# mjlaine/mcmcf90

Measured on AMD Instinct MI355X. Metric: MH proposals/sec (whole node), d=50 Gaussian target, higher is better.
Workload: dtype f64

## Files before the change

### mcmcf90_amd/csrc/mcx_api.hip

```cpp
#include <hip/hip_runtime.h>
#include <csignal>
#include <cmath>
#include <cstdio>
#include <cstdlib>
#include <cstring>
#include <string>
#include <vector>
#include <algorithm>
#include "../../include/mcmcx.h"
#include "../../include/mcmcx_target.h"
#include "mcx_kernels.hpp"
#include "mcx_group.hpp"
#include "mcx_group_ram.hpp"

#include "mcx_host_engine.hpp"
#include "mcx_host_linalg.hpp"
#include "mcx_host_launch.hpp"
#include "mcx_host_adapt.hpp"
#include "mcx_host_pooled.hpp"
#include "mcx_host_callbacks.hpp"

extern "C" {

const char *mcmcx_last_error(void) { return g_err.c_str(); }
// ... 316 lines not shown
    E.ny = h->ny; E.hs = h->d + h->ny;
    E.alphatarget = c.alphatarget; E.drscale = c.drscale; E.scalelimit = c.scalelimit; E.scalefactor = c.scalefactor;
    E.k0 = c.seed; E.chain_id0 = c.chain_id0;
    E.dr_lds = h->plan.dr_lds ? 1 : 0;
    E.lds_scratch = h->plan.lds_form;
    E.tgt.kind = phased(h) ? (int)TGT_HOST : h->tkind;
    E.tgt.b = h->tb; E.tgt.ndata = (int)h->tx.size(); E.tgt.ncols = h->tncols;
    const int d = h->d;
    int rc;
    if (h->tkind == TGT_GAUSS) {
        if ((rc = dev_upload(h, &E.tgt.mu, h->tmu))) return rc;
        std::vector<double> lt((size_t)(d + 4) * d + 64, 0.0);
        for (int i = 0; i < d; ++i) for (int j = 0; j < d; ++j) lt[(size_t)j * d + i] = h->tlam[(size_t)i * d + j];
        if ((rc = dev_upload(h, &E.tgt.lamT, lt))) return rc;
    }
    if (h->tkind == TGT_EXPDATA || h->tkind == TGT_EXPCOLS) { if ((rc = dev_upload(h, &E.tgt.x, h->tx))) return rc; if ((rc = dev_upload(h,
        &E.tgt.y, h->ty))) return rc; }
    if (h->has_lo && (rc = dev_upload(h, &E.tgt.lo, h->tlo))) return rc;
    if (h->has_hi && (rc = dev_upload(h, &E.tgt.hi, h->thi))) return rc;
    if (h->has_pri) { if ((rc = dev_upload(h, &E.tgt.pmu, h->tpmu))) return rc; if ((rc = dev_upload(h, &E.tgt.psig, h->tpsig))) return rc;
        }
    if ((rc = dev_upload(h, &E.par0, h->par0))) return rc;
    return dev_upload(h, &E.cmat0p, f.Cp);
}
static int init_chains(mcmcx_engine *h, const InitialFactor &f)
{
    const mcmcx_config &c = h->cfg;
    EngineDev &E = h->E;
    const int d = h->d, P = h->P, T = h->ntiles, ny = h->ny;
    const size_t L = (size_t)T * 64, DD = (size_t)d * d;
    int rc;
    if ((rc = dev_alloc(h, &E.theta, L * d))) return rc;
    if ((rc = h->plan.host_mapped ? host_alloc(h, &E.cand, L * d) : dev_alloc(h, &E.cand, L * d))) return rc;
    if ((rc = dev_alloc(h, &E.zs, L * 2 * d))) return rc;
    if ((rc = h->plan.cs_mapped ? host_alloc(h, &E.cs, L * 2 * d) : dev_alloc(h, &E.cs, L * 2 * d))) return rc;
    if (h->plan.xscr && (rc = dev_alloc(h, &E.xscr, L * 2 * d))) return rc;
    if ((rc = dev_alloc(h, &E.scal, L * NSCAL))) return rc;
    if ((rc = dev_alloc(h, &E.ictr, L * NICTR))) return rc;
    if ((rc = dev_alloc(h, &E.rngn, L))) return rc;
    if (!h->pooled && (rc = dev_alloc(h, &E.R, L * P, false))) return rc;
    if ((rc = dev_alloc(h, &E.basetheta, L * d))) return rc;
    if (h->usesvd && !h->pooled) {
        if ((rc = dev_alloc(h, &E.Rf, L * DD, false))) return rc;
        if (c.method != MCMCX_METHOD_RAM) {
            if ((rc = dev_alloc(h, &E.Gw, L * DD)) || (rc = dev_alloc(h, &E.Vw, L * DD))) return rc;
            if (h->plan.svd_blocked && ((rc = dev_alloc(h, &h->d_Gc, L * DD, false)) || (rc = dev_alloc(h, &h->d_Vc, L * DD, false))
                || (rc = dev_alloc(h, &h->d_svc, L * d, false)) || (rc = dev_alloc(h, &h->d_need, L)) || (rc = dev_alloc(h, &h->d_state, L))
                || (rc = dev_alloc(h, &h->d_anyrot, 1)))) return rc;
        }
        if ((rc = dev_alloc(h, &E.qstd, L * d))) return rc;
        if (h->dodr && (rc = dev_alloc(h, &E.R2f, L * DD, false))) return rc;
        if ((rc = dev_bcast(h, E.Rf, f.Rfull)) || (rc = dev_bcast(h, E.qstd, f.qstd))) return rc;
        if (h->dodr) {
            std::vector<double> r2 = f.Rfull;
            for (auto &v : r2) v = v / c.drscale;
            if ((rc = dev_bcast(h, E.R2f, r2))) return rc;
        }
    }
    if (h->dodr && !h->pooled && ((rc = dev_alloc(h, &E.R2, L * P, false)) || (rc = dev_alloc(h, &E.iC, L * P, false)))) return rc;
    const bool am = h->plan.am;
    h->wcap = 0;
    if (am || c.record_chain) {
        long long wc = (c.record_chain || (am && c.adapthist > 1)) ? (long long)c.nsimu + 1
                                      : (long long)c.burnintime + 2LL * c.adaptint + c.adapthist + 2;
        if (wc > (long long)c.nsimu + 1) wc = (long long)c.nsimu + 1;
        h->wcap = (int)wc;
        if ((rc = dev_alloc(h, &E.hist, L * (size_t)h->wcap * (d + ny), false))) return rc;
        if ((rc = dev_alloc(h, &E.wacc, (size_t)T * h->wcap))) return rc;
        if (c.record_chain && c.updatesigma) { E.record_s2 = 1; if ((rc = dev_alloc(h, &E.s2hist, L * (size_t)h->wcap * ny))) return rc; }
// ... 675 lines not shown
```

### mcmcf90_amd/csrc/mcx_common.hpp

```cpp
#pragma once
#include "mcx_device.hpp"
#include <type_traits>

namespace mcx {


enum { TGT_GAUSS = 0, TGT_BANANA = 1, TGT_EXPDATA = 2, TGT_HOST = 3, TGT_EXPCOLS = 4, TGT_MODULE = 5 };
enum { M_DRAM = 0, M_RAM = 1, M_ER = 3 };

enum { S_SS1 = 0, S_PRI1, S_SIGMA2, S_ALPHA12, S_SAVEDY, S_WSUM, S_WNEW, NSCAL };
enum { I_SAVED = 0, I_STAYED, I_BNDSTAYED, I_DRACC, I_DRTRIES, I_CHAININD, I_CURCOUNT, I_STATUS,
       I_LASTFREQ, I_BASECNT, I_WINSTART, I_INFO, I_ERSTAYED, I_PDESC, I_DOWNS, I_ADFLAGS, I_NR, I_BSTART, NICTR };

enum { ST_RAM_DOWNDATE_FAIL = 1, ST_CHOL_FAIL = 2, ST_POTRI_FAIL = 4 };

struct DevTarget {
    int kind;
    const double *mu, *lamT;
    double b;
    int ndata;
    const double *x, *y;
    int ncols;
    const double *lo, *hi;
    const double *pmu, *psig;
};

struct EngineDev {
    int d, P, ntiles;
    int method, dodr, updatesigma, doadapt, doburnin, burnintime, greedy, adapthist;
    double initcmatn;
    double gam_shape;
    double N0S02;
    double alphatarget, drscale, scalelimit, scalefactor;
    DevTarget tgt;
    double *theta, *cand, *zs, *cs, *scal, *R, *R2, *iC, *Rtmp;
    double *xscr;
    double *cmat, *mean, *basetheta;
    const double *cmat0p, *par0;
    uint32_t *ictr;
    uint64_t *rngn;
    uint32_t k0, chain_id0;
    int wcap, record_s2;
    double *hist, *s2hist;
    uint64_t *wacc;
    uint64_t *accmask;
    uint64_t *rowlist;
    const double *sharedR;
    int usesvd, doscam; double condmax;
    int scam_fast;
    double *Rf, *R2f, *qstd, *Gw, *Vw;
    double *hev, *hx;
    int ny, hs;
    double *ssv, *s2v, *ss2v;
    const double *gshapev;
    int lds_scratch;
    int dr_lds;
};

#define TIDX(base, tile, K, k, lane) ((base)[((size_t)(tile) * (size_t)(K) + (size_t)(k)) * 64 + (lane)])

MCX_DEV int rowstart(int i, int d) { return i * d - (i * (i - 1)) / 2; }
MCX_DEV int pidx(int i, int j, int d) { return rowstart(i, d) + (j - i); }

constexpr int CH = 8;

#define XL(j) X[(j) * 64 + lane]
#define GV(p, k) (p)[(size_t)(k) * 64 + lane]
#define GV2(p, k, c) (p)[(size_t)(k) * 64 + (c)]
#define LDNT(p, k) __builtin_nontemporal_load(&(p)[(size_t)(k) * 64 + lane])
// ... 423 lines not shown
```

### mcmcf90_amd/csrc/mcx_host_engine.hpp

```cpp

using namespace mcx;
static_assert(MCMCX_HE_INB == HE_INB && MCMCX_HE_PRI == HE_PRI && MCMCX_HE_SS == HE_SS && MCMCX_HX_STAGE2 == HX_STAGE2
    && MCMCX_HX_CRIT == HX_CRIT,
              "include/mcmcx_target.h and mcx_kernels.hpp disagree about the phase-state slots");

static thread_local std::string g_err;
static int fail(int code, const std::string &msg) { g_err = msg; return code; }

#define HIPCHK(call)                                                                              \
    do {                                                                                          \
        hipError_t e_ = (call);                                                                   \
        if (e_ != hipSuccess)                                                                     \
            return fail(-100, std::string(#call) + ": " + hipGetErrorString(e_));                 \
    } while (0)

struct mcx_switches {
    int pooled_mfma_dr_min = -1, pooled_scalar = -1, dr_big = -1, scam_pooled_16 = -1, scam_fast_lanes = -1, scam_waves = -1,
        svd_lane = -1, cov_batch_rows = -1, ram_wide = -1, pooled_waves = -1, pooled_ks = -1, cols_phased = -1, host_mapped = -1,
            host_fuse = -1, lds_scratch = -1, group = -1, group_dr2 = -1, group_gw = -1, ram_group = -1, tile_factor = -1,
            pooled_phase_mfma = -1;
    static int get(const char *name) { const char *e = getenv(name); return e ? atoi(e) : -1; }
    void read()
    {
        pooled_mfma_dr_min = get("MCMCX_POOLED_MFMA_DR_MIN"); pooled_scalar = get("MCMCX_POOLED_SCALAR"); dr_big = get("MCMCX_DR_BIG");
        scam_pooled_16 = get("MCMCX_SCAM_POOLED_16"); scam_fast_lanes = get("MCMCX_SCAM_FAST_LANES");
        scam_waves = get("MCMCX_SCAM_WAVES"); svd_lane = get("MCMCX_SVD_LANE"); cov_batch_rows = get("MCMCX_COV_BATCH_ROWS");
        ram_wide = get("MCMCX_RAM_WIDE"); pooled_waves = get("MCMCX_POOLED_WAVES"); pooled_ks = get("MCMCX_POOLED_KS");
        cols_phased = get("MCMCX_COLS_PHASED"); host_mapped = get("MCMCX_HOST_MAPPED"); host_fuse = get("MCMCX_HOST_FUSE");
        lds_scratch = get("MCMCX_LDS_SCRATCH"); group = get("MCMCX_GROUP"); group_dr2 = get("MCMCX_GROUP_DR2");
        group_gw = get("MCMCX_GROUP_GW"); ram_group = get("MCMCX_RAM_GROUP"); tile_factor = get("MCMCX_TILE_FACTOR");
        pooled_phase_mfma = get("MCMCX_POOLED_PHASE_MFMA");
    }
};
enum LdsForm { LDS_NONE = 0, LDS_STATE = 1, LDS_STATE_R = 2, LDS_RAM_R = 3 };
enum SharedLayout { SH_R = 1, SH_RT = 2, SH_DR = 4, SH_DRT = 8, SH_U = 16, SH_UREP = 32 };
struct KernelEntry;
struct KernelPlan {
    int lds_form = LDS_NONE;
    bool dr_lds = false;
    bool dr_vectors_in_lds = false;
    int group_d4 = 0, group_drm = 0, group_gw = 16;
    int ram_group_d4 = 0;
    bool tile_factor = false;
    bool svd_blocked = false;
    bool cov_batch = true;
    bool scam_replicated = false;
    bool host_mapped = false, cs_mapped = false;
    bool host_fuse = true;
    bool fused_cols = false;
    bool pooled_mfma = false;
    bool pooled_dr_mfma = false;
    bool pooled_two_waves = false, pooled_forty_rows = false;
    int pooled_phase = 0;
    bool ram_wide = false;
    bool scam_pooled12 = false, scam_fast_tile = false; int scam_waves = 1;
    bool am = false;
    bool xscr = false;
    unsigned shared = 0;
    const KernelEntry *step = nullptr;
    const KernelEntry *scam = nullptr;
};
struct PooledState {
    int status = 0; double alpha = 0.0;
    double W = 0.0; std::vector<double> mean, C, R;
    std::vector<double> Rf;
    std::vector<double> U, std;
    std::vector<double> R2, iC;
    double *d_R = nullptr;
    double *d_RT = nullptr;
    double *d_R2 = nullptr, *d_iC = nullptr;
    double *d_R2T = nullptr, *d_iCd = nullptr;
    double *d_U = nullptr;
};
struct mcmcx_engine {
    mcmcx_config cfg;
    KernelPlan plan;
    int d = 0, P = 0, ntiles = 0, nlanes = 0;
    int dodr = 0, usesvd = 0;
    bool inited = false;
    int simuind = 0;
    const char *last_kernel = "";
    std::string launch_err;
    std::vector<double> par0, cmat0;
    double sigma2 = 1.0; int nobs = 1; bool sigma2ok = false;
    int ny = 1; std::vector<double> sigma2v; std::vector<int> nobsv;
    int tkind = -1, tncols = 1; std::vector<double> tmu, tlam, tx, ty, tlo, thi, tpmu, tpsig; double tb = 0.1;
    bool has_lo = false, has_hi = false, has_pri = false;
// ... 94 lines not shown
```

### mcmcf90_amd/csrc/mcx_host_launch.hpp

```cpp

static size_t pooled_mfma_lds(int d)
{
    const size_t d4 = (size_t)((d + 3) & ~3), nt = (size_t)((d + 15) / 16);
    const size_t rows = (nt <= 4) ? std::max(d4, 4 * nt) : d4 + 16 * nt + 4 * nt;
    return rows * 64 * sizeof(double);
}
static bool pooled_use_mfma(const mcmcx_engine *h, const mcx_switches &sw)
{
    if (!h->pooled || (h->cfg.method != MCMCX_METHOD_DRAM && h->cfg.method != MCMCX_METHOD_RAM
        && h->cfg.method != MCMCX_METHOD_ER)) return false;
    if (h->dodr) {
        int dmin = 21;
        if (sw.pooled_mfma_dr_min >= 0) dmin = sw.pooled_mfma_dr_min;
        if (h->d < dmin) return false;
    }
    if (sw.pooled_scalar > 0) return false;
    return pooled_mfma_lds(h->d) <= 160 * 1024;
}
static bool phased(const mcmcx_engine *h) { return h->tkind == TGT_HOST || h->tkind == TGT_EXPCOLS || h->tkind == TGT_MODULE; }
static bool phase_cut(const mcmcx_engine *h) { return phased(h) && !h->plan.fused_cols; }
static int kernel_method(const mcmcx_engine *h)
{
    const int m = h->cfg.method;
    return (m == MCMCX_METHOD_RAM && !h->pooled) ? M_RAM : (m == MCMCX_METHOD_ER ? M_ER : M_DRAM);
}
static size_t lds_bytes(const mcmcx_engine *h) { return (size_t)h->d * 64 * sizeof(double) * 2; }
static bool dr_fits_lds(const mcmcx_engine *h) { return lds_bytes(h) <= 160 * 1024; }
static size_t lds_step(const mcmcx_engine *h) { return h->plan.dr_lds ? lds_bytes(h) : 0; }
static bool dr_vectors_in_lds(const mcmcx_engine *h, const mcx_switches &sw, int min_waves)
{
    if (!dr_fits_lds(h)) return false;
    if (sw.dr_big >= 0) return sw.dr_big == 0;
    return lds_bytes(h) * (size_t)min_waves <= 160 * 1024;
}
static void launch_init(mcmcx_engine *h)
{ hipLaunchKernelGGL(init_kernel, dim3(h->ntiles), dim3(64), 0, h->stream, h->E); }
struct KernelEntry {
    const char *family;
    const char *name;
    bool (*when)(const mcmcx_engine *);
    void (*launch)(mcmcx_engine *, int it0, int it1);
    unsigned shared = 0;
};
static const KernelEntry *pick_entry(const mcmcx_engine *h, const KernelEntry *tab, size_t n)
{
    for (size_t i = 0; i < n; ++i)
        if (tab[i].when(h)) return &tab[i];
    return nullptr;
}
static void launch_entry(mcmcx_engine *h, const KernelEntry *e, const char *family, int it0, int it1)
{
    if (!e) { h->launch_err = std::string("no ") + family + " kernel covers this configuration"; return; }
    h->last_kernel = e->name;
    e->launch(h, it0, it1);
}
static const int GROUP_MAXSEG = 256;
static const int GROUP_MAX_NPAR = 64, GROUP_MAX_NPAR_DR = 32;
static bool group_covers(const mcmcx_engine *h)
{
    const mcmcx_config &c = h->cfg;
    return !h->pooled && (c.method == MCMCX_METHOD_DRAM || (c.method == MCMCX_METHOD_ER && !h->dodr)) && !h->usesvd && !phased(h)
        && h->ny == 1 &&
           (h->tkind == TGT_GAUSS || h->tkind == TGT_BANANA || h->tkind == TGT_EXPDATA) && h->d <= (h->dodr ? GROUP_MAX_NPAR_DR
               : GROUP_MAX_NPAR) &&
           !(h->tkind == TGT_BANANA && h->d < 2) && !(h->tkind == TGT_EXPDATA && h->d < 2);
}
static int group_width(const mcmcx_engine *h)
{
    if ((long long)h->cfg.nchains <= 16384 || h->d > 16 || h->cfg.updatesigma) return 16;
    if (!h->dodr) return 4;
    return h->d <= 8 ? 4 : 16;
}
static bool group_wins(const mcmcx_engine *h, int drm, int gw)
{
    const long long n = h->cfg.nchains;
// ... 167 lines not shown
         h->pool.d_RT, h->pool.d_R2T, h->pool.d_iCd); }, SH_RT | SH_DRT},
    MCX_VARIANT_STEP_ENTRIES
    {"step", "pooled_mfma_ks_kernel", [](const mcmcx_engine *h) { return h->plan.pooled_forty_rows; },
     [](mcmcx_engine *h, int it0, int it1) {
         const size_t lds = (size_t)PKS * 64 * sizeof(double);
         if (((h->d + 3) & ~3) == 52) hipLaunchKernelGGL(pooled_mfma_ks_kernel<true>, G1, lds, STEP_ARGS, STEP_TGT, h->pool.d_RT);
         else hipLaunchKernelGGL(pooled_mfma_ks_kernel<false>, G1, lds, STEP_ARGS, STEP_TGT, h->pool.d_RT); }, SH_RT},
    {"step", "pooled_mfma_kernel<false, true>", [](const mcmcx_engine *h) {
        return h->plan.pooled_mfma && h->plan.pooled_two_waves; },
     [](mcmcx_engine *h, int it0, int it1) { hipLaunchKernelGGL((pooled_mfma_kernel<false, true>), G1, pooled_mfma_lds(h->d), STEP_ARGS,
         STEP_TGT, h->pool.d_RT, (const double *)nullptr, (const double *)nullptr); }, SH_RT},
    {"step", "pooled_mfma_kernel<false>", [](const mcmcx_engine *h) { return h->plan.pooled_mfma; },
     [](mcmcx_engine *h, int it0, int it1) { hipLaunchKernelGGL(pooled_mfma_kernel<false>, G1, pooled_mfma_lds(h->d), STEP_ARGS, STEP_TGT,
         h->pool.d_RT, (const double *)nullptr, (const double *)nullptr); }, SH_RT},
    {"step", "step_kernel_pooled_dr_big", [](const mcmcx_engine *h) { return h->pooled && h->dodr && !h->plan.dr_vectors_in_lds; },
     [](mcmcx_engine *h, int it0, int it1) { hipLaunchKernelGGL(step_kernel_pooled_dr_big, G1, 0, STEP_ARGS, STEP_RS, STEP_TGT,
         h->E.sharedR, h->pool.d_R2, h->pool.d_iC); }, SH_R | SH_DR},
    {"step", "step_kernel_pooled_dr", [](const mcmcx_engine *h) { return h->pooled && h->dodr; },
     [](mcmcx_engine *h, int it0, int it1) { hipLaunchKernelGGL(step_kernel_pooled_dr, G1, lds_step(h), STEP_ARGS, STEP_RS, STEP_TGT,
         h->E.sharedR, h->pool.d_R2, h->pool.d_iC); }, SH_R | SH_DR},
    {"step", "step_kernel<false, false, true>", [](const mcmcx_engine *h) { return h->pooled != 0; },
     [](mcmcx_engine *h, int it0, int it1) { hipLaunchKernelGGL((step_kernel<false, false, true>), G1, 0, STEP_ARGS, STEP_RS, STEP_TGT,
         h->E.sharedR); }, SH_R},
    {"step", "group_ram_kernel", [](const mcmcx_engine *h) { return h->plan.ram_group_d4 != 0; }, launch_group_ram},
    {"step", "step_kernel_ram_fullr", [](const mcmcx_engine *h) { return kernel_method(h) == M_RAM && h->usesvd; },
     [](mcmcx_engine *h, int it0, int it1) { hipLaunchKernelGGL(step_kernel_ram_fullr, G1, 0, STEP_ARGS, STEP_RS, STEP_TGT, h->E.sharedR);
         }},
    {"step", "step_kernel_ram_ldsr", [](const mcmcx_engine *h) {
        return kernel_method(h) == M_RAM && h->plan.lds_form == LDS_RAM_R; },
     [](mcmcx_engine *h, int it0, int it1) { hipLaunchKernelGGL(step_kernel_ram_ldsr, G1, (size_t)(2 * h->d + h->P) * 64 * sizeof(double),
         STEP_ARGS, STEP_RS, STEP_TGT, h->E.sharedR); }},
    {"step", "step_kernel_ram_wide", [](const mcmcx_engine *h) {
        return kernel_method(h) == M_RAM && h->d > RAM_SMALL_MAX && h->plan.ram_wide; },
     [](mcmcx_engine *h, int it0, int it1) { hipLaunchKernelGGL(step_kernel_ram_wide, G1, (size_t)NLC * 2 * 64 * sizeof(double), STEP_ARGS,
         STEP_RS, STEP_TGT, h->E.sharedR); }},
    {"step", "step_kernel<true, false, false>", [](const mcmcx_engine *h) { return kernel_method(h) == M_RAM; },
     [](mcmcx_engine *h, int it0, int it1) { hipLaunchKernelGGL((step_kernel<true, false, false>), G1,
         (size_t)NLC * 2 * 64 * sizeof(double), STEP_ARGS, STEP_RS, STEP_TGT, h->E.sharedR); }},
    {"step", "step_kernel_dr_big", [](const mcmcx_engine *h) { return h->dodr && !h->plan.dr_vectors_in_lds; },
     [](mcmcx_engine *h, int it0, int it1) { hipLaunchKernelGGL(step_kernel_dr_big, G1, 0, STEP_ARGS, STEP_TGT); }},
    {"step", "step_kernel_dr", [](const mcmcx_engine *h) { return h->dodr != 0; },
     [](mcmcx_engine *h, int it0, int it1) { hipLaunchKernelGGL(step_kernel_dr, G1, lds_step(h), STEP_ARGS, STEP_TGT); }},
    {"step", "step_kernel_ldsr", [](const mcmcx_engine *h) { return h->plan.lds_form == LDS_STATE_R; },
     [](mcmcx_engine *h, int it0, int it1) { hipLaunchKernelGGL(step_kernel_ldsr, G1, (size_t)(2 * h->d + h->P) * 64 * sizeof(double),
         STEP_ARGS, STEP_RS, STEP_TGT, h->E.sharedR); }},
    {"step", "step_kernel_ldsv", [](const mcmcx_engine *h) { return h->plan.lds_form != LDS_NONE; },
     [](mcmcx_engine *h, int it0, int it1) { hipLaunchKernelGGL(step_kernel_ldsv, G1, (size_t)4 * h->d * 64 * sizeof(double), STEP_ARGS,
         STEP_RS, STEP_TGT, h->E.sharedR); }},
    {"step", "step_kernel<false, false, false>", [](const mcmcx_engine *) { return true; },
     [](mcmcx_engine *h, int it0, int it1) { hipLaunchKernelGGL((step_kernel<false, false, false>), G1, 0, STEP_ARGS, STEP_RS, STEP_TGT,
         h->E.sharedR); }},
};
static void launch_step(mcmcx_engine *h, int it0, int it1)
{
    if (h->plan.group_d4) launch_group(h, it0, it1);
    else launch_entry(h, h->plan.step, "step", it0, it1);
}
static int dev_bcast(mcmcx_engine *h, double *dst, const std::vector<double> &v)
{
    double *tmp = nullptr;
    HIPCHK(hipMalloc(&tmp, v.size() * sizeof(double)));
    hipError_t e = hipMemcpy(tmp, v.data(), v.size() * sizeof(double), hipMemcpyHostToDevice);
    if (e == hipSuccess) {
        const unsigned gy = (unsigned)std::min<size_t>(v.size(), 64);
        hipLaunchKernelGGL(bcast_kernel, dim3(h->ntiles, gy), dim3(64), 0, h->stream, dst, tmp, v.size());
        e = hipGetLastError();
        if (e == hipSuccess) e = hipStreamSynchronize(h->stream);
    }
// ... 108 lines not shown
    p.host_fuse = sw.host_fuse != 0;
    p.scam_replicated = h->usesvd && h->pooled && c.method == MCMCX_METHOD_SCAM && (scam_pooled_lds(d) > 160 * 1024 || pphase);
    p.pooled_mfma = pooled_use_mfma(h, sw) && !pphase;
    p.pooled_dr_mfma = p.pooled_mfma && h->dodr;
    p.pooled_two_waves = pooled_two_waves(h, sw);
    p.pooled_forty_rows = pooled_forty_rows(h, sw);
    p.ram_wide = sw.ram_wide != 0;
    p.scam_pooled12 = scam_use_12(h, sw);
    p.scam_fast_tile = scam_fast_tile_kernel(h, sw);
    p.scam_waves = scam_tile_waves(h, sw);
    if (group_covers(h)) {
        int ex = 0;
        const bool pow2 = h->dodr && c.drscale > 0.0 && std::frexp(c.drscale, &ex) == 0.5 && ex > -64 && ex < 64;
        const int drm = !h->dodr ? 0 : (pow2 && d <= 24 && sw.group_dr2 != 0) ? 2 : 1;
        const int gw = (d <= 16 && sw.group_gw != -1) ? (sw.group_gw == 4 ? 4 : 16) : group_width(h);
        if (sw.group != -1 ? sw.group != 0 : group_wins(h, drm, gw)) {
            p.group_d4 = d <= 32 ? ((d + 3) & ~3) : ((d + 7) & ~7);
            p.group_gw = gw;
            p.group_drm = drm;
        }
    }
    if (ram_group_covers(h)) {
        const int rg = sw.ram_group != -1 ? sw.ram_group : sw.group;
        if (rg != -1 ? rg != 0 : ram_group_wins(h)) p.ram_group_d4 = d <= 16 ? 16 : d <= 32 ? 32 : d <= 56 ? 56 : 64;
    }
    p.tile_factor = am && !h->usesvd && d <= (sw.tile_factor == 1 ? 64 : 32) && sw.tile_factor != 0;
    p.svd_blocked = svd_blocked(h, sw) && (c.doadapt != 0 || c.doburnin != 0);
    p.cov_batch = !(sw.cov_batch_rows > 0);
    if (pphase) (c.method == MCMCX_METHOD_SCAM ? p.scam : p.step) = pick_entry(h, PHASE_TABLE,
        sizeof(PHASE_TABLE) / sizeof(PHASE_TABLE[0]));
    else if (c.method == MCMCX_METHOD_SCAM) p.scam = pick_entry(h, SCAM_TABLE, sizeof(SCAM_TABLE) / sizeof(SCAM_TABLE[0]));
    else if (p.group_d4) p.step = pick_entry(h, GROUP_TABLE, sizeof(GROUP_TABLE) / sizeof(GROUP_TABLE[0]));
    else p.step = pick_entry(h, STEP_TABLE, sizeof(STEP_TABLE) / sizeof(STEP_TABLE[0]));
    const KernelEntry *e = c.method == MCMCX_METHOD_SCAM ? p.scam : p.step;
    p.shared = (h->pooled && e) ? e->shared & (h->dodr ? ~0u : ~(unsigned)(SH_DR | SH_DRT)) : 0;
    if (h->usesvd && (p.shared & SH_R)) p.shared ^= SH_R | SH_RT;
}
```

### mcmcf90_amd/csrc/mcx_step.hpp

```cpp
#pragma once
#include "mcx_products.hpp"

namespace mcx {

#ifndef MCX_NLC
#define MCX_NLC 19
#endif
#ifndef MCX_MIXED_UNROLL
#define MCX_MIXED_UNROLL 1
#endif
#ifndef MCX_RAM_WAVES
#define MCX_RAM_WAVES 2
#endif
constexpr int NLC = MCX_NLC;
template <bool MIXED, int RWT = RW>
MCX_DEV bool ram_update(double *Rt, const double *zc_t, const double *zn_t, double *cs_t, double *P_t,
                        const double *theta_t, int lane, int d, double a, double su, bool act, bool fuse, uint32_t &status,
                        double *lc, bool &pdesc)
{
    const bool up = act && (a >= 0.0);
    const bool down = act && !(a >= 0.0);
    const int rwe = (RWT == RW) ? RW : ram_panel_width(d, RWT);
#define CS_(k, w) (*((lc && (k) < NLC) ? &lc[(2 * (k) + (w)) * 64 + lane] : &cs_t[(size_t)(2 * (k) + (w)) * 64 + lane]))
    if (__any(act)) {
        if (act) {
            for (int J0 = 0; J0 < d; J0 += rwe) {
                const int nw = (d - J0) < rwe ? (d - J0) : rwe;
                double xa[RWT], P[RWT];
#pragma unroll
                for (int u = 0; u < RWT; ++u) { xa[u] = up ? GV(zc_t, J0 + (u < nw ? u : nw - 1)) / su * a : 0.0; P[u] = 0.0; }
if (MIXED) {
                    double rn[RWT], cn = 0.0, sn_ = 0.0, zn_ = 0.0;
                    if (J0 > 0) {
                        const double *sg = Rt + (size_t)J0 * 64;
#pragma unroll
                        for (int u = 0; u < RWT; ++u) rn[u] = LDNT(sg, u < nw ? u : nw - 1);
                        sn_ = CS_(0, 1);
                        if (up) { cn = CS_(0, 0); zn_ = fuse ? GV(zn_t, 0) : 0.0; }
                    }
#pragma unroll MCX_MIXED_UNROLL
                    for (int i = 0; i < J0; ++i) {
                        double *seg = Rt + (size_t)(rowstart(i, d) + J0 - i) * 64;
                        double r[RWT];
#pragma unroll
                        for (int u = 0; u < RWT; ++u) r[u] = rn[u];
                        const double c = cn, sn = sn_, zi = zn_;
                        if (i + 1 < J0) {
                            const double *sg = Rt + (size_t)(rowstart(i + 1, d) + J0 - (i + 1)) * 64;
#pragma unroll
                            for (int u = 0; u < RWT; ++u) rn[u] = LDNT(sg, u < nw ? u : nw - 1);
                            sn_ = CS_(i + 1, 1);
                            if (up) { cn = CS_(i + 1, 0); zn_ = fuse ? GV(zn_t, i + 1) : 0.0; }
                        }
                        if (up) {
#pragma unroll
                            for (int u = 0; u < RWT; ++u) {
                                double t = c * r[u] + sn * xa[u];
                                xa[u] = c * xa[u] - sn * r[u];
                                r[u] = t;
                                P[u] = dfma(t, zi, P[u]);
                            }
                        } else {
#pragma unroll
                            for (int u = 0; u < RWT; ++u) xa[u] = dfma(r[u], sn, xa[u]);
                        }
#pragma unroll
                        for (int u = 0; u < RWT; ++u) if (u < nw) STNT(seg, u, r[u]);
                    }
                } else {
#pragma unroll 2
                    for (int i = 0; i < J0; ++i) {
                        double *seg = Rt + (size_t)(rowstart(i, d) + J0 - i) * 64;
                        double r[RWT];
#pragma unroll
                        for (int u = 0; u < RWT; ++u) r[u] = LDNT(seg, u < nw ? u : nw - 1);
                        if (up) {
                            const bool inl = lc && i < NLC;
                            const double c = inl ? lc[(2 * i) * 64 + lane] : GV(cs_t, 2 * i);
                            const double sn = inl ? lc[(2 * i + 1) * 64 + lane] : GV(cs_t, 2 * i + 1);
                            const double zi = fuse ? GV(zn_t, i) : 0.0;
#pragma unroll
                            for (int u = 0; u < RWT; ++u) {
                                double t = c * r[u] + sn * xa[u];
                                xa[u] = c * xa[u] - sn * r[u];
                                if (u < nw) STNT(seg, u, t);
                                P[u] = dfma(t, zi, P[u]);
                            }
                        } else {
                            const double si = CS_(i, 1);
#pragma unroll
                            for (int u = 0; u < RWT; ++u) xa[u] = dfma(r[u], si, xa[u]);
                        }
                    }
                }
                for (int i = J0; i < J0 + nw; ++i) {
                    double *seg = Rt + (size_t)rowstart(i, d) * 64;
                    const int ui = i - J0, m = d - 1 - i;
                    double r[RWT];
#pragma unroll
                    for (int u = 0; u < RWT; ++u) { int k = u - ui; k = k < 0 ? 0 : k; k = k > m ? m : k; r[u] = LDNT(seg, k); }
                    double xi = xa[0];
#pragma unroll
                    for (int u = 1; u < RWT; ++u) xi = (u == ui) ? xa[u] : xi;
                    if (up) {
                        const double zi = fuse ? GV(zn_t, i) : 0.0;
                        double rr, c, sn;
                        d_rotg(GV(seg, 0), xi, rr, c, sn);
                        GV(seg, 0) = rr;
                        if (lc && i < NLC) { lc[(2 * i) * 64 + lane] = c; lc[(2 * i + 1) * 64 + lane] = sn; }
                        else if (J0 + nw < d) { GV(cs_t, 2 * i) = c; GV(cs_t, 2 * i + 1) = sn; }
#pragma unroll
                        for (int u = 0; u < RWT; ++u) {
                            const bool off = (u > ui) && (u < nw);
                            double t = c * r[u] + sn * xa[u];
                            double nx = c * xa[u] - sn * r[u];
                            xa[u] = off ? nx : xa[u];
                            if (!MIXED) { if (off) STNT(seg, u - ui, t); }
                            else r[u] = off ? t : r[u];
                            double tp = (u == ui) ? rr : t;
                            double np = dfma(tp, zi, P[u]);
                            P[u] = (u >= ui && u < nw) ? np : P[u];
                        }
                    } else {
                        double si = -(GV(zc_t, i) / su * a) - xi;
                        si = si / GV(seg, 0);
                        CS_(i, 1) = si;
#pragma unroll
                        for (int u = 0; u < RWT; ++u) { double na = dfma(r[u], si, xa[u]); xa[u] = (u > ui) ? na : xa[u]; }
                    }
                    if (MIXED) {
#pragma unroll
                        for (int u = 0; u < RWT; ++u) if ((u > ui) && (u < nw)) STNT(seg, u - ui, r[u]);
                    }
                }
                if (up && fuse) {
                    double th[RWT];
#pragma unroll
                    for (int u = 0; u < RWT; ++u) th[u] = GV(theta_t, J0 + (u < nw ? u : nw - 1));
#pragma unroll
                    for (int u = 0; u < RWT; ++u) if (u < nw) GV(P_t, J0 + u) = th[u] + P[u];
                }
            }
        }
    }
    if (up) pdesc = false;
    bool down_ok = false;
    if (__any(down)) {
        if (down) {
            double norm;
            if (d == 1) norm = fabs(CS_(0, 1));
// ... 99 lines not shown
                        }
                    } else {
#pragma unroll 2
                        for (int i = J0 - 1; i >= 0; --i) {
                            double *seg = Rt + (size_t)(rowstart(i, d) + J0 - i) * 64;
                            const double ci = CS_(i, 0), si = CS_(i, 1);
                            const double zi = fuse ? GV(zn_t, i) : 0.0;
                            double r[RWT];
#pragma unroll
                            for (int u = 0; u < RWT; ++u) r[u] = LDB(seg, u < nw ? u : nw - 1);
#pragma unroll
                            for (int u = 0; u < RWT; ++u) {
                                double t = ci * xx[u] + si * r[u];
                                const double nr = ci * r[u] - si * xx[u];
                                if (u < nw) STB(seg, u, nr);
                                xx[u] = t;
                                P[u] = dfma(nr, zi, P[u]);
                            }
                        }
                    }
                    if (fuse && down_ok) {
                        double th[RWT];
#pragma unroll
                        for (int u = 0; u < RWT; ++u) th[u] = GV(theta_t, J0 + (u < nw ? u : nw - 1));
#pragma unroll
                        for (int u = 0; u < RWT; ++u) if (u < nw) GV(P_t, J0 + u) = th[u] + P[u];
                    }
                }
            }
        }
    }
    return (up || down_ok) && fuse;
#undef CS_
}

#define RF(i, j) Rf_t[((size_t)(j) * d + (i)) * 64 + lane]
MCX_DEV void ram_update_full(double *Rf_t, const double *zc_t, double *cs_t, int lane, int d, double a, double su, bool act,
                             uint32_t &status)
{
    if (!act) return;
    if (a >= 0.0) {
        for (int j = 0; j < d; ++j) {
            double xj = GV(zc_t, j) / su * a;
            for (int i = 0; i < j; ++i) {
                const double c = GV(cs_t, 2 * i), sn = GV(cs_t, 2 * i + 1), r = RF(i, j);
                double t = c * r + sn * xj;
                xj = c * xj - sn * r;
                RF(i, j) = t;
            }
            double rr, c, sn;
            d_rotg(RF(j, j), xj, rr, c, sn);
            RF(j, j) = rr; GV(cs_t, 2 * j) = c; GV(cs_t, 2 * j + 1) = sn;
        }
        return;
    }
    for (int j = 0; j < d; ++j) {
        double acc = 0.0;
        for (int i = 0; i < j; ++i) acc = dfma(RF(i, j), GV(cs_t, 2 * i + 1), acc);
        double xj = -(GV(zc_t, j) / su * a);
        double sj = xj - acc;
        GV(cs_t, 2 * j + 1) = sj / RF(j, j);
    }
    double norm;
    if (d == 1) norm = fabs(GV(cs_t, 1));
    else {
        double scale = 0.0, ssq = 1.0;
// ... 83 lines not shown
    extern __shared__ double Xlds[];
    const int lane = threadIdx.x, tile = blockIdx.x, d = E.d;
    double *X = XG ? E.xscr + (size_t)tile * 2 * d * 64 : Xlds;
    constexpr bool ldsv = LDSV && !RAM && !DR && !POOLED;
    constexpr bool ldsr = ldsv && LDSR;
    double *theta_g = E.theta + (size_t)tile * d * 64;
    double *theta_t = ldsv ? X : theta_g;
    double *cand_t = ldsv ? X + (size_t)d * 64 : E.cand + (size_t)tile * d * 64;
    double *zs_t = ldsr ? cand_t : (ldsv ? X + (size_t)2 * d * 64 : E.zs + (size_t)tile * 2 * d * 64);
    double *cs_t = E.cs + (size_t)tile * 2 * d * 64;
    if (ldsv) for (int k = 0; k < d; ++k) GV(theta_t, k) = GV(theta_g, k);
    constexpr bool ramr = RAM && LDSR && !FULLR;
    double *Rt = (ldsr || ramr) ? X + (size_t)2 * d * 64 : E.R + (size_t)tile * E.P * 64;
    if (ldsr || ramr) { const double *Rg = E.R + (size_t)tile * E.P * 64; copy_vec(Rt, Rg, nullptr, lane, E.P); }
    double *Y = X + (size_t)d * 64;
    double *c2_t = cs_t;

    Rng g;
    g.k0 = E.k0; g.k1 = E.chain_id0 + (uint32_t)(tile * 64 + lane);
    g.n = TIDX(E.rngn, tile, 1, 0, lane); g.cblk = 0; g.c2 = 0; g.c3 = 0;
    g.saved = (int)TIDX(E.ictr, tile, NICTR, I_SAVED, lane);
    g.saved_y = TIDX(E.scal, tile, NSCAL, S_SAVEDY, lane);
    double ss1 = TIDX(E.scal, tile, NSCAL, S_SS1, lane), pri1 = TIDX(E.scal, tile, NSCAL, S_PRI1, lane);
    double sigma2 = TIDX(E.scal, tile, NSCAL, S_SIGMA2, lane), alpha12 = TIDX(E.scal, tile, NSCAL, S_ALPHA12, lane);
    uint32_t stayed = TIDX(E.ictr, tile, NICTR, I_STAYED, lane), bnd = TIDX(E.ictr, tile, NICTR, I_BNDSTAYED, lane);
    uint32_t chainind = TIDX(E.ictr, tile, NICTR, I_CHAININD, lane), curcount = TIDX(E.ictr, tile, NICTR, I_CURCOUNT, lane);
    uint32_t status = TIDX(E.ictr, tile, NICTR, I_STATUS, lane);
    uint32_t dracc = TIDX(E.ictr, tile, NICTR, I_DRACC, lane), drtries = TIDX(E.ictr, tile, NICTR, I_DRTRIES, lane);
    uint32_t erstayed = TIDX(E.ictr, tile, NICTR, I_ERSTAYED, lane);
    bool pdesc = RAM && TIDX(E.ictr, tile, NICTR, I_PDESC, lane) != 0u;
    uint32_t downs = RAM ? TIDX(E.ictr, tile, NICTR, I_DOWNS, lane) : 0u;

    bool have_p = false;
    double su_c = gen_normals<RAM ? 1 : MCX_RNG_NB>(g, zs_t + (ldsr ? 0 : (size_t)(it0 & 1) * d * 64), lane, d, true), su_n = 0.0;

    for (int it = it0; it <= it1; ++it) {
        double *zc_t = ldsr ? zs_t : zs_t + (size_t)(it & 1) * d * 64;
        double *zn_t = ldsr ? zs_t : zs_t + (size_t)((it + 1) & 1) * d * 64;
        if (POOLED) { if (E.usesvd) gemvN_shared(g_sharedR, zc_t, cand_t, theta_t, lane, d); else trmv_shared(g_sharedR, zc_t, cand_t,
            theta_t, lane, d); }
        else if (E.usesvd) gemvN_panels(E.Rf + (size_t)tile * d * d * 64, zc_t, cand_t, theta_t, lane, d, true);
        else if (__any(!have_p)) trmv_panels<!RAM>(Rt, zc_t, cand_t, theta_t, lane, d, !have_p, RAM && pdesc);
        bool inb = target_inbounds(E.tgt, d, lane, cand_t);
        double pri2 = target_prior(E.tgt, d, lane, cand_t);
        double ss2 = target_ss<WIDE_T>(E.tgt, d, lane, cand_t, g_mu, g_lamT);
        bool reject;
        if (!RAM && !DR && E.method == M_ER) {
            if (!inb) { bnd += 1; reject = true; }
            else {
                double u = rng_uniform(g);
                double sscrit = -2.0 * d_log(u) + ss1 / sigma2 + pri1;
                if (pri2 >= sscrit) { reject = true; erstayed += 1; }
                else { sscrit = sigma2 * (sscrit - pri2); reject = (ss2 >= sscrit); }
            }
        } else if (!inb) {
            if (!DR) bnd += 1;
            reject = true;
            if (!RAM) alpha12 = 0.0;
        } else {
            alpha12 = d_alpha(ss1, pri1, ss2, pri2, sigma2);
            reject = true;
            if (alpha12 >= 1.0) reject = false;
            else if (alpha12 > 0.0) { double u = rng_uniform(g); if (u <= alpha12) reject = false; }
        }
        bool dr_moved = false;
        if (DR && __any(reject)) {
            const bool m = reject;
            if (m) drtries += 1;
            double *z2_t = zn_t;
            gen_normals<RAM ? 1 : MCX_RNG_NB>(g, z2_t, lane, d, m);
            if (POOLED) {
// ... 19 lines not shown
                    double qb = POOLED ? quadform_sym_shared(g_sharediC, lane, d, X, Y) : quadform_sym(iCt, lane, d, X, Y);
                    double q1 = -0.5 * (qa - qb);
                    double alpha13 = min1(d_exp(l2 + q1) * (1.0 - alpha32) / (1.0 - alpha12));
                    bool rej2 = true;
                    if (alpha13 >= 1.0) rej2 = false;
                    else if (alpha13 > 0.0) { double u = rng_uniform(g); if (u <= alpha13) rej2 = false; }
                    if (!rej2) { dracc += 1; reject = false; dr_moved = true; ss2 = ss3; pri2 = pri3; }
                }
            }
        }
        if (reject) { stayed += 1; curcount += 1; }
        else { ss1 = ss2; pri1 = pri2; chainind += 1; curcount = 1; }
        if (E.updatesigma) {
            double gm = rng_gamma(g, E.gam_shape, 2.0 / (E.N0S02 + ss1));
            sigma2 = 1.0 / gm;
        }
        unsigned long long ballot = __ballot(!reject);
        const int slot = it % E.wcap;
        if (!reject) {
            double *h = E.hist ? E.hist + ((size_t)tile * E.wcap + slot) * (size_t)E.hs * 64 : nullptr;
            const double *src = dr_moved ? c2_t : cand_t;
            copy_vec(theta_t, src, h, lane, d);
            if (h) GV(h, d) = ss1;
        }
        if (E.hist) {
            if (lane == 0) E.wacc[(size_t)tile * E.wcap + slot] = ballot;
            if (E.record_s2) E.s2hist[((size_t)tile * E.wcap + slot) * 64 + lane] = sigma2;
        }
        if (E.accmask && lane == 0) E.accmask[(size_t)(it - 1) * E.ntiles + tile] = ballot;
        const bool pre = (it < it1);
        if (pre) su_n = gen_normals<RAM ? 1 : MCX_RNG_NB>(g, zn_t, lane, d, true);
        have_p = false;
        if (RAM && E.doadapt != 0 && !(it < E.burnintime && E.doburnin != 0)) {
            double a = ramscale[it - it0] * (alpha12 - E.alphatarget);
            downs += (a >= 0.0) ? 0u : 1u;
            if (FULLR) ram_update_full(E.Rf + (size_t)tile * d * d * 64, zc_t, cs_t, lane, d, a, su_c, true, status);
            else if (__any(!(a >= 0.0)))
                have_p = ram_update<true, RWT>(Rt, zc_t, zn_t, cs_t, cand_t, theta_t, lane, d, a, su_c, true, pre, status,
                    RAM ? X : nullptr, pdesc);
            else have_p = ram_update<false, RWT>(Rt, zc_t, zn_t, cs_t, cand_t, theta_t, lane, d, a, su_c, true, pre, status,
                RAM ? X : nullptr, pdesc);
        }
        su_c = su_n;
    }

    TIDX(E.rngn, tile, 1, 0, lane) = g.n;
    TIDX(E.ictr, tile, NICTR, I_SAVED, lane) = (uint32_t)g.saved;
    TIDX(E.scal, tile, NSCAL, S_SAVEDY, lane) = g.saved_y;
    TIDX(E.scal, tile, NSCAL, S_SS1, lane) = ss1; TIDX(E.scal, tile, NSCAL, S_PRI1, lane) = pri1;
    TIDX(E.scal, tile, NSCAL, S_SIGMA2, lane) = sigma2; TIDX(E.scal, tile, NSCAL, S_ALPHA12, lane) = alpha12;
    TIDX(E.ictr, tile, NICTR, I_STAYED, lane) = stayed; TIDX(E.ictr, tile, NICTR, I_BNDSTAYED, lane) = bnd;
    TIDX(E.ictr, tile, NICTR, I_CHAININD, lane) = chainind; TIDX(E.ictr, tile, NICTR, I_CURCOUNT, lane) = curcount;
    TIDX(E.ictr, tile, NICTR, I_STATUS, lane) = status;
    TIDX(E.ictr, tile, NICTR, I_DRACC, lane) = dracc; TIDX(E.ictr, tile, NICTR, I_DRTRIES, lane) = drtries;
    TIDX(E.ictr, tile, NICTR, I_ERSTAYED, lane) = erstayed;
    if (RAM) { TIDX(E.ictr, tile, NICTR, I_PDESC, lane) = pdesc ? 1u : 0u; TIDX(E.ictr, tile, NICTR, I_DOWNS, lane) = downs; }
    if (ldsv) for (int k = 0; k < d; ++k) GV(theta_g, k) = GV(theta_t, k);
    if (ramr) { double *Rg = E.R + (size_t)tile * E.P * 64; copy_vec(Rg, Rt, nullptr, lane, E.P); }
}


constexpr int TQ = 10;
MCX_DEV void quadform2_panels(const double *St, int lane, int d, const double *Xa, const double *Xb, double *ysa, double *ysb,
                              double &qa, double &qb)
{
    qa = 0.0; qb = 0.0;
    for (int J0 = 0; J0 < d; J0 += TQ) {
        const int nw = (d - J0) < TQ ? (d - J0) : TQ;
        const bool last = J0 + TQ >= d;
        double Ya[TQ], Yb[TQ], xja[TQ], xjb[TQ];
#pragma unroll
        for (int u = 0; u < TQ; ++u) { const int j = J0 + (u < nw ? u : nw - 1); xja[u] = GV(Xa, j); xjb[u] = GV(Xb, j); Ya[u] = 0.0;
            Yb[u] = 0.0; }
        {
#ifndef MCX_Q2_NB
// ... 214 lines not shown
```

Measured before the change: 222.3 million.

## Fuse consecutive RAM Cholesky rank-one updates into a single pass over R

Adds a paired RAM update path for the wide RAM step kernel. When every lane's update is an up-date, the Cholesky factor is not written back; the Givens factors are kept and the next iteration applies both rotations in one sweep over R. This is meant to halve the global load and store traffic on the per-chain factor. It adds a third normal-vector slot, extra rotation buffers and LDS, and more complex control logic that changes the floating-point ordering.

```diff
diff --git a/mcmcf90_amd/csrc/mcx_api.hip b/mcmcf90_amd/csrc/mcx_api.hip
--- a/mcmcf90_amd/csrc/mcx_api.hip
+++ b/mcmcf90_amd/csrc/mcx_api.hip
@@ -372,9 +372,10 @@
     int rc;
     if ((rc = dev_alloc(h, &E.theta, L * d))) return rc;
     if ((rc = h->plan.host_mapped ? host_alloc(h, &E.cand, L * d) : dev_alloc(h, &E.cand, L * d))) return rc;
-    if ((rc = dev_alloc(h, &E.zs, L * 2 * d))) return rc;
+    if ((rc = dev_alloc(h, &E.zs, L * (h->plan.ram_pair ? 3 : 2) * d))) return rc;
     if ((rc = h->plan.cs_mapped ? host_alloc(h, &E.cs, L * 2 * d) : dev_alloc(h, &E.cs, L * 2 * d))) return rc;
     if (h->plan.xscr && (rc = dev_alloc(h, &E.xscr, L * 2 * d))) return rc;
+    if (h->plan.ram_pair && (rc = dev_alloc(h, &E.pr, L * 2 * d))) return rc;
     if ((rc = dev_alloc(h, &E.scal, L * NSCAL))) return rc;
     if ((rc = dev_alloc(h, &E.ictr, L * NICTR))) return rc;
     if ((rc = dev_alloc(h, &E.rngn, L))) return rc;
diff --git a/mcmcf90_amd/csrc/mcx_common.hpp b/mcmcf90_amd/csrc/mcx_common.hpp
--- a/mcmcf90_amd/csrc/mcx_common.hpp
+++ b/mcmcf90_amd/csrc/mcx_common.hpp
@@ -35,6 +35,7 @@
     DevTarget tgt;
     double *theta, *cand, *zs, *cs, *scal, *R, *R2, *iC, *Rtmp;
     double *xscr;
+    double *pr;
     double *cmat, *mean, *basetheta;
     const double *cmat0p, *par0;
     uint32_t *ictr;
diff --git a/mcmcf90_amd/csrc/mcx_host_engine.hpp b/mcmcf90_amd/csrc/mcx_host_engine.hpp
--- a/mcmcf90_amd/csrc/mcx_host_engine.hpp
+++ b/mcmcf90_amd/csrc/mcx_host_engine.hpp
@@ -18,7 +18,7 @@
     int pooled_mfma_dr_min = -1, pooled_scalar = -1, dr_big = -1, scam_pooled_16 = -1, scam_fast_lanes = -1, scam_waves = -1,
         svd_lane = -1, cov_batch_rows = -1, ram_wide = -1, pooled_waves = -1, pooled_ks = -1, cols_phased = -1, host_mapped = -1,
             host_fuse = -1, lds_scratch = -1, group = -1, group_dr2 = -1, group_gw = -1, ram_group = -1, tile_factor = -1,
-            pooled_phase_mfma = -1;
+            pooled_phase_mfma = -1, ram_pair = -1;
     static int get(const char *name) { const char *e = getenv(name); return e ? atoi(e) : -1; }
     void read()
     {
@@ -29,7 +29,7 @@
         cols_phased = get("MCMCX_COLS_PHASED"); host_mapped = get("MCMCX_HOST_MAPPED"); host_fuse = get("MCMCX_HOST_FUSE");
         lds_scratch = get("MCMCX_LDS_SCRATCH"); group = get("MCMCX_GROUP"); group_dr2 = get("MCMCX_GROUP_DR2");
         group_gw = get("MCMCX_GROUP_GW"); ram_group = get("MCMCX_RAM_GROUP"); tile_factor = get("MCMCX_TILE_FACTOR");
-        pooled_phase_mfma = get("MCMCX_POOLED_PHASE_MFMA");
+        pooled_phase_mfma = get("MCMCX_POOLED_PHASE_MFMA"); ram_pair = get("MCMCX_RAM_PAIR");
     }
 };
 enum LdsForm { LDS_NONE = 0, LDS_STATE = 1, LDS_STATE_R = 2, LDS_RAM_R = 3 };
@@ -53,6 +53,7 @@
     bool pooled_two_waves = false, pooled_forty_rows = false;
     int pooled_phase = 0;
     bool ram_wide = false;
+    bool ram_pair = false;
     bool scam_pooled12 = false, scam_fast_tile = false; int scam_waves = 1;
     bool am = false;
     bool xscr = false;
diff --git a/mcmcf90_amd/csrc/mcx_host_launch.hpp b/mcmcf90_amd/csrc/mcx_host_launch.hpp
--- a/mcmcf90_amd/csrc/mcx_host_launch.hpp
+++ b/mcmcf90_amd/csrc/mcx_host_launch.hpp
@@ -41,6 +41,7 @@
     bool (*when)(const mcmcx_engine *);
     void (*launch)(mcmcx_engine *, int it0, int it1);
     unsigned shared = 0;
+    bool ram_pair = false;
 };
 static const KernelEntry *pick_entry(const mcmcx_engine *h, const KernelEntry *tab, size_t n)
 {
@@ -274,8 +275,9 @@
          STEP_ARGS, STEP_RS, STEP_TGT, h->E.sharedR); }},
     {"step", "step_kernel_ram_wide", [](const mcmcx_engine *h) {
         return kernel_method(h) == M_RAM && h->d > RAM_SMALL_MAX && h->plan.ram_wide; },
-     [](mcmcx_engine *h, int it0, int it1) { hipLaunchKernelGGL(step_kernel_ram_wide, G1, (size_t)NLC * 2 * 64 * sizeof(double), STEP_ARGS,
-         STEP_RS, STEP_TGT, h->E.sharedR); }},
+     [](mcmcx_engine *h, int it0, int it1) { hipLaunchKernelGGL(step_kernel_ram_wide, G1, (size_t)(NLC * 2 + 2) * 64 * sizeof(double),
+         STEP_ARGS,
+         STEP_RS, STEP_TGT, h->E.sharedR); }, 0, true},
     {"step", "step_kernel<true, false, false>", [](const mcmcx_engine *h) { return kernel_method(h) == M_RAM; },
      [](mcmcx_engine *h, int it0, int it1) { hipLaunchKernelGGL((step_kernel<true, false, false>), G1,
          (size_t)NLC * 2 * 64 * sizeof(double), STEP_ARGS, STEP_RS, STEP_TGT, h->E.sharedR); }},
@@ -450,6 +452,7 @@
     else if (c.method == MCMCX_METHOD_SCAM) p.scam = pick_entry(h, SCAM_TABLE, sizeof(SCAM_TABLE) / sizeof(SCAM_TABLE[0]));
     else if (p.group_d4) p.step = pick_entry(h, GROUP_TABLE, sizeof(GROUP_TABLE) / sizeof(GROUP_TABLE[0]));
     else p.step = pick_entry(h, STEP_TABLE, sizeof(STEP_TABLE) / sizeof(STEP_TABLE[0]));
+    p.ram_pair = sw.ram_pair != 0 && p.step && p.step->ram_pair;
     const KernelEntry *e = c.method == MCMCX_METHOD_SCAM ? p.scam : p.step;
     p.shared = (h->pooled && e) ? e->shared & (h->dodr ? ~0u : ~(unsigned)(SH_DR | SH_DRT)) : 0;
     if (h->usesvd && (p.shared & SH_R)) p.shared ^= SH_R | SH_RT;
diff --git a/mcmcf90_amd/csrc/mcx_step.hpp b/mcmcf90_amd/csrc/mcx_step.hpp
--- a/mcmcf90_amd/csrc/mcx_step.hpp
+++ b/mcmcf90_amd/csrc/mcx_step.hpp
@@ -13,11 +13,12 @@
 #define MCX_RAM_WAVES 2
 #endif
 constexpr int NLC = MCX_NLC;
-template <bool MIXED, int RWT = RW>
+template <bool MIXED, int RWT = RW, int PEEK = 0>
 MCX_DEV bool ram_update(double *Rt, const double *zc_t, const double *zn_t, double *cs_t, double *P_t,
                         const double *theta_t, int lane, int d, double a, double su, bool act, bool fuse, uint32_t &status,
-                        double *lc, bool &pdesc)
+                        double *lc, bool &pdesc, bool wr = true)
 {
+    const bool st = PEEK == 0 ? true : PEEK == 1 ? false : wr;
     const bool up = act && (a >= 0.0);
     const bool down = act && !(a >= 0.0);
     const int rwe = (RWT == RW) ? RW : ram_panel_width(d, RWT);
@@ -83,7 +84,7 @@
                             for (int u = 0; u < RWT; ++u) {
                                 double t = c * r[u] + sn * xa[u];
                                 xa[u] = c * xa[u] - sn * r[u];
-                                if (u < nw) STNT(seg, u, t);
+                                if (st) { if (u < nw) STNT(seg, u, t); }
                                 P[u] = dfma(t, zi, P[u]);
                             }
                         } else {
@@ -106,7 +107,7 @@
                         const double zi = fuse ? GV(zn_t, i) : 0.0;
                         double rr, c, sn;
                         d_rotg(GV(seg, 0), xi, rr, c, sn);
-                        GV(seg, 0) = rr;
+                        if (st) GV(seg, 0) = rr;
                         if (lc && i < NLC) { lc[(2 * i) * 64 + lane] = c; lc[(2 * i + 1) * 64 + lane] = sn; }
                         else if (J0 + nw < d) { GV(cs_t, 2 * i) = c; GV(cs_t, 2 * i + 1) = sn; }
 #pragma unroll
@@ -115,7 +116,7 @@
                             double t = c * r[u] + sn * xa[u];
                             double nx = c * xa[u] - sn * r[u];
                             xa[u] = off ? nx : xa[u];
-                            if (!MIXED) { if (off) STNT(seg, u - ui, t); }
+                            if (!MIXED) { if (st && off) STNT(seg, u - ui, t); }
                             else r[u] = off ? t : r[u];
                             double tp = (u == ui) ? rr : t;
                             double np = dfma(tp, zi, P[u]);
@@ -281,6 +282,93 @@
     }
     return (up || down_ok) && fuse;
 #undef CS_
+}
+
+#ifndef MCX_RW_PAIR
+#define MCX_RW_PAIR 13
+#endif
+#ifndef MCX_NL2
+#define MCX_NL2 (MCX_NLC / 2)
+#endif
+constexpr int RW_PAIR = MCX_RW_PAIR, NL2 = MCX_NL2;
+template <int W2>
+MCX_DEV void ram_update2(double *Rt, const double *z1_t, const double *z2_t, const double *zn_t, double *cs1_t, double *cs2_t,
+                         double *P_t, const double *theta_t, int lane, int d, double a1, double su1, double a2, double su2, bool fuse,
+                         double *lc)
+{
+    const int rwe = ram_panel_width(d, W2);
+    double *lc2 = lc + (size_t)2 * NL2 * 64;
+    for (int J0 = 0; J0 < d; J0 += rwe) {
+        const int nw = (d - J0) < rwe ? (d - J0) : rwe;
+        double xa1[W2], xa2[W2], P[W2];
+#pragma unroll
+        for (int u = 0; u < W2; ++u) {
+            const int j = J0 + (u < nw ? u : nw - 1);
+            xa1[u] = GV(z1_t, j) / su1 * a1; xa2[u] = GV(z2_t, j) / su2 * a2; P[u] = 0.0;
+        }
+#define MCX_P2_ROW(c1_, s1_, c2_, s2_) { \
+            double *seg = Rt + (size_t)(rowstart(i, d) + J0 - i) * 64; \
+            double r[W2]; \
+            _Pragma("unroll") for (int u = 0; u < W2; ++u) r[u] = LDNT(seg, u < nw ? u : nw - 1); \
+            const double c1 = (c1_), s1 = (s1_), c2 = (c2_), s2 = (s2_); \
+            const double zi = fuse ? GV(zn_t, i) : 0.0; \
+            _Pragma("unroll") for (int u = 0; u < W2; ++u) { \
+                const double t1 = c1 * r[u] + s1 * xa1[u]; \
+                xa1[u] = c1 * xa1[u] - s1 * r[u]; \
+                const double t2 = c2 * t1 + s2 * xa2[u]; \
+                xa2[u] = c2 * xa2[u] - s2 * t1; \
+                if (u < nw) STNT(seg, u, t2); \
+                P[u] = dfma(t2, zi, P[u]); \
+            } }
+        const int nl = J0 < NL2 ? J0 : NL2;
+        for (int i = 0; i < nl; ++i)
+            MCX_P2_ROW(lc[(2 * i) * 64 + lane], lc[(2 * i + 1) * 64 + lane], lc2[(2 * i) * 64 + lane], lc2[(2 * i + 1) * 64 + lane])
+        for (int i = nl; i < J0; ++i)
+            MCX_P2_ROW(GV(cs1_t, 2 * i), GV(cs1_t, 2 * i + 1), GV(cs2_t, 2 * i), GV(cs2_t, 2 * i + 1))
+#undef MCX_P2_ROW
+        for (int i = J0; i < J0 + nw; ++i) {
+            double *seg = Rt + (size_t)rowstart(i, d) * 64;
+            const int ui = i - J0, m = d - 1 - i;
+            double r[W2];
+#pragma unroll
+            for (int u = 0; u < W2; ++u) { int k = u - ui; k = k < 0 ? 0 : k; k = k > m ? m : k; r[u] = LDNT(seg, k); }
+            double xi1 = xa1[0], xi2 = xa2[0], r0 = r[0];
+#pragma unroll
+            for (int u = 1; u < W2; ++u) { xi1 = (u == ui) ? xa1[u] : xi1; xi2 = (u == ui) ? xa2[u] : xi2; r0 = (u == ui) ? r[u] : r0; }
+            const double zi = fuse ? GV(zn_t, i) : 0.0;
+            double rr1, c1, s1, rr2, c2, s2;
+            d_rotg(r0, xi1, rr1, c1, s1);
+            d_rotg(rr1, xi2, rr2, c2, s2);
+            GV(seg, 0) = rr2;
+            if (J0 + nw < d) {
+                if (i < NL2) {
+                    lc[(2 * i) * 64 + lane] = c1; lc[(2 * i + 1) * 64 + lane] = s1;
+                    lc2[(2 * i) * 64 + lane] = c2; lc2[(2 * i + 1) * 64 + lane] = s2;
+                } else { GV(cs1_t, 2 * i) = c1; GV(cs1_t, 2 * i + 1) = s1; GV(cs2_t, 2 * i) = c2; GV(cs2_t, 2 * i + 1) = s2; }
+            }
+#pragma unroll
+            for (int u = 0; u < W2; ++u) {
+                const bool off = (u > ui) && (u < nw);
+                const double t1 = c1 * r[u] + s1 * xa1[u];
+                const double n1 = c1 * xa1[u] - s1 * r[u];
+                const double t2 = c2 * t1 + s2 * xa2[u];
+                const double n2 = c2 * xa2[u] - s2 * t1;
+                xa1[u] = off ? n1 : xa1[u];
+                xa2[u] = off ? n2 : xa2[u];
+                if (off) STNT(seg, u - ui, t2);
+                const double tp = (u == ui) ? rr2 : t2;
+                const double np = dfma(tp, zi, P[u]);
+                P[u] = (u >= ui && u < nw) ? np : P[u];
+            }
+        }
+        if (fuse) {
+            double th[W2];
+#pragma unroll
+            for (int u = 0; u < W2; ++u) th[u] = GV(theta_t, J0 + (u < nw ? u : nw - 1));
+#pragma unroll
+            for (int u = 0; u < W2; ++u) if (u < nw) GV(P_t, J0 + u) = th[u] + P[u];
+        }
+    }
 }
 
 #define RF(i, j) Rf_t[((size_t)(j) * d + (i)) * 64 + lane]
@@ -430,11 +518,18 @@
     uint32_t downs = RAM ? TIDX(E.ictr, tile, NICTR, I_DOWNS, lane) : 0u;
 
     bool have_p = false;
-    double su_c = gen_normals<RAM ? 1 : MCX_RNG_NB>(g, zs_t + (ldsr ? 0 : (size_t)(it0 & 1) * d * 64), lane, d, true), su_n = 0.0;
+    constexpr bool PAIR = RAM && !FULLR && !LDSR && RWT != RW;
+    const bool pair_on = PAIR && E.pr != nullptr;
+    if (pair_on) zs_t = E.zs + (size_t)tile * 3 * d * 64;
+    double *cs2_t = PAIR ? E.pr + (size_t)tile * 2 * d * 64 : nullptr;
+    bool pend = false;
+    int zslot = pair_on ? it0 % 3 : (it0 & 1);
+    double su_c = gen_normals<RAM ? 1 : MCX_RNG_NB>(g, zs_t + (ldsr ? 0 : (size_t)zslot * d * 64), lane, d, true), su_n = 0.0;
 
     for (int it = it0; it <= it1; ++it) {
-        double *zc_t = ldsr ? zs_t : zs_t + (size_t)(it & 1) * d * 64;
-        double *zn_t = ldsr ? zs_t : zs_t + (size_t)((it + 1) & 1) * d * 64;
+        const int zslot_n = pair_on ? (zslot == 2 ? 0 : zslot + 1) : (zslot ^ 1);
+        double *zc_t = ldsr ? zs_t : zs_t + (size_t)zslot * d * 64;
+        double *zn_t = ldsr ? zs_t : zs_t + (size_t)zslot_n * d * 64;
         if (POOLED) { if (E.usesvd) gemvN_shared(g_sharedR, zc_t, cand_t, theta_t, lane, d); else trmv_shared(g_sharedR, zc_t, cand_t,
             theta_t, lane, d); }
         else if (E.usesvd) gemvN_panels(E.Rf + (size_t)tile * d * d * 64, zc_t, cand_t, theta_t, lane, d, true);
@@ -520,15 +615,42 @@
         if (pre) su_n = gen_normals<RAM ? 1 : MCX_RNG_NB>(g, zn_t, lane, d, true);
         have_p = false;
         if (RAM && E.doadapt != 0 && !(it < E.burnintime && E.doburnin != 0)) {
-            double a = ramscale[it - it0] * (alpha12 - E.alphatarget);
+            const double a = ramscale[it - it0] * (alpha12 - E.alphatarget);
             downs += (a >= 0.0) ? 0u : 1u;
             if (FULLR) ram_update_full(E.Rf + (size_t)tile * d * d * 64, zc_t, cs_t, lane, d, a, su_c, true, status);
+            else if (PAIR) {
+                enum { J_CUR, J_MAT, J_DOUBLE };
+                const bool allup = !__any(!(a >= 0.0));
+                const bool peek = pair_on && allup && pre && !pend;
+                const double *zp_t = zs_t + (size_t)(zslot_n == 2 ? 0 : zslot_n + 1) * d * 64;
+                double a_p = 0.0, su_p = 0.0;
+                if (pend) { a_p = X[(2 * NLC) * 64 + lane]; su_p = X[(2 * NLC + 1) * 64 + lane]; }
+                for (int job = pend ? (allup ? J_DOUBLE : J_MAT) : J_CUR;; job = J_CUR) {
+                    if (job == J_DOUBLE) {
+                        ram_update2<RW_PAIR>(Rt, zp_t, zc_t, zn_t, cs_t, cs2_t, cand_t, theta_t, lane, d, a_p, su_p, a, su_c, pre, X);
+                        have_p = pre; pdesc = false;
+                        break;
+                    }
+                    const bool mat = (job == J_MAT);
+                    if (!mat && !allup) {
+                        have_p = ram_update<true, RWT>(Rt, zc_t, zn_t, cs_t, cand_t, theta_t, lane, d, a, su_c, true, pre, status, X,
+                            pdesc);
+                        break;
+                    }
+                    have_p = ram_update<false, RWT, 2>(Rt, mat ? zp_t : zc_t, zn_t, cs_t, cand_t, theta_t, lane, d,
+                        mat ? a_p : a, mat ? su_p : su_c, true, mat ? false : pre, status, X, pdesc, mat || !peek);
+                    if (!mat) break;
+                }
+                pend = peek;
+                if (peek) { X[(2 * NLC) * 64 + lane] = a; X[(2 * NLC + 1) * 64 + lane] = su_c; }
+            }
             else if (__any(!(a >= 0.0)))
                 have_p = ram_update<true, RWT>(Rt, zc_t, zn_t, cs_t, cand_t, theta_t, lane, d, a, su_c, true, pre, status,
                     RAM ? X : nullptr, pdesc);
             else have_p = ram_update<false, RWT>(Rt, zc_t, zn_t, cs_t, cand_t, theta_t, lane, d, a, su_c, true, pre, status,
                 RAM ? X : nullptr, pdesc);
         }
+        zslot = zslot_n;
         su_c = su_n;
     }
 
```

Result: faster. 239.9 million, median of 6 (+7.9%).
